# seanome/kmerseek

Hardware: AMD Instinct MI355X
Metric: k-mers hashed+matched/sec (higher is better)
Workload: dtype u64

## Files before the change

### include/kmerseek_amd.h

```cpp
#ifndef KMERSEEK_AMD_H
#define KMERSEEK_AMD_H

#include <stddef.h>
#include <stdint.h>

#ifdef __cplusplus
extern "C" {
#endif

#define KS_ABI_VERSION 1

typedef enum ks_status {
    KS_OK = 0,
    KS_ERR_INVALID_MOLTYPE = 1,
    KS_ERR_INVALID_KSIZE = 2,
    KS_ERR_INVALID_RESIDUE = 3,
    KS_ERR_INVALID_ARG = 4,
    KS_ERR_OOM = 5,
    KS_ERR_HIP = 6,
    KS_ERR_NO_DEVICE = 7,
    KS_ERR_CAPACITY = 8,
    KS_ERR_INVALID_SCALED = 9
} ks_status;

// ... 26 lines not shown
const char *ks_status_string(int status);

int ks_moltype_from_string(const char *name, uint32_t *moltype_out);

uint64_t ks_max_hash(uint32_t scaled);

int ks_ctx_create(int device, void *hip_stream, ks_ctx **out);
void ks_ctx_destroy(ks_ctx *ctx);
const char *ks_last_error(const ks_ctx *ctx);
void *ks_ctx_stream(const ks_ctx *ctx);
int ks_ctx_synchronize(ks_ctx *ctx);
int ks_ctx_pool_stats(const ks_ctx *ctx, uint64_t *n_blocks, uint64_t *bytes_held, uint64_t *bytes_in_use,
                      uint64_t *n_mallocs);

int ks_ctx_sketch_stats(const ks_ctx *ctx, uint64_t out[4]);
int ks_ctx_search_stats(const ks_ctx *ctx, uint64_t out[4]);
int ks_ctx_fused_stats(const ks_ctx *ctx, uint64_t out[3]);
int ks_ctx_qfilter_stats(const ks_ctx *ctx, uint64_t out[2]);
int ks_ctx_reload_debug_env(ks_ctx *ctx);
int ks_debug_guard_selftest(const char *what);

int ks_dev_malloc(ks_ctx *ctx, uint64_t bytes, void **out);
int ks_dev_free(ks_ctx *ctx, void *ptr);
int ks_dev_upload(ks_ctx *ctx, void *dst_device, const void *src_host, uint64_t bytes);
int ks_dev_download(ks_ctx *ctx, void *dst_host, const void *src_device, uint64_t bytes);

int ks_host_alloc(ks_ctx *ctx, uint64_t bytes, void **out);
int ks_host_free(ks_ctx *ctx, void *ptr);


typedef struct ks_residue_error {
    uint32_t seq_index;
// ... 535 lines not shown
```

### kmerseek_amd/_lib.py

```python
from __future__ import annotations

import ctypes as C
import os
import sys

HERE = os.path.dirname(os.path.abspath(__file__))
SO_PATH = os.environ.get("KMERSEEK_AMD_LIB") or os.path.join(HERE, "libkmerseek_amd.so")

KS_OK = 0
KS_ERR_INVALID_MOLTYPE = 1
KS_ERR_INVALID_KSIZE = 2
KS_ERR_INVALID_RESIDUE = 3
KS_ERR_INVALID_ARG = 4
KS_ERR_OOM = 5
KS_ERR_HIP = 6
KS_ERR_NO_DEVICE = 7
KS_ERR_CAPACITY = 8
KS_ERR_INVALID_SCALED = 9

KS_PROTEIN, KS_DAYHOFF, KS_HP = 0, 1, 2
KS_SEED_DEFAULT = 42


class ks_params(C.Structure):
# ... 119 lines not shown
_u64p = C.POINTER(C.c_uint64)
_pp = C.POINTER(C.c_void_p)
_parp = C.POINTER(ks_params)

SIGNATURES = {
    "ks_abi_version": (C.c_uint32, []),
    "ks_status_string": (C.c_char_p, [C.c_int]),
    "ks_moltype_from_string": (C.c_int, [C.c_char_p, _u32p]),
    "ks_max_hash": (C.c_uint64, [C.c_uint32]),
    "ks_ctx_create": (C.c_int, [C.c_int, _vp, _pp]),
    "ks_ctx_destroy": (None, [_vp]),
    "ks_last_error": (C.c_char_p, [_vp]),
    "ks_ctx_stream": (_vp, [_vp]),
    "ks_ctx_synchronize": (C.c_int, [_vp]),
    "ks_ctx_sketch_stats": (C.c_int, [_vp, C.POINTER(C.c_uint64 * 4)]),
    "ks_ctx_search_stats": (C.c_int, [_vp, C.POINTER(C.c_uint64 * 4)]),
    "ks_ctx_fused_stats": (C.c_int, [_vp, C.POINTER(C.c_uint64 * 3)]),
    "ks_ctx_qfilter_stats": (C.c_int, [_vp, C.POINTER(C.c_uint64 * 2)]),
    "ks_ctx_reload_debug_env": (C.c_int, [_vp]),
    "ks_debug_guard_selftest": (C.c_int, [C.c_char_p]),
    "ks_host_alloc": (C.c_int, [_vp, C.c_uint64, _pp]),
    "ks_host_free": (C.c_int, [_vp, _vp]),
    "ks_dev_malloc": (C.c_int, [_vp, C.c_uint64, _pp]),
    "ks_dev_free": (C.c_int, [_vp, _vp]),
    "ks_dev_upload": (C.c_int, [_vp, _vp, _vp, C.c_uint64]),
    "ks_dev_download": (C.c_int, [_vp, _vp, _vp, C.c_uint64]),
    "ks_ctx_pool_stats": (C.c_int, [_vp, _u64p, _u64p, _u64p, _u64p]),
    "ks_validate_and_resolve": (C.c_int, [C.c_char_p, C.c_uint64, C.c_int, C.c_uint64, C.c_char_p, _u64p,
                                          C.POINTER(ks_residue_error)]),
    "ks_sketch_batch": (C.c_int, [_vp, _vp, _vp, C.c_uint32, _parp, _pp]),
    "ks_sketch_batch_device": (C.c_int, [_vp, _vp, _vp, C.c_uint32, C.c_uint64, C.c_uint32, _parp, _pp]),
    "ks_sketch_queries_device": (C.c_int, [_vp, _vp, _vp, _vp, C.c_uint32, C.c_uint64, C.c_uint32, _pp]),
# ... 302 lines not shown
```

### kmerseek_amd/csrc/ks_api.hip

```cpp
#include "ks_device.h"

extern "C" int ks_sketch_batch_device(ks_ctx *ctx, const uint8_t *d_residues, const uint64_t *d_seq_offsets,
                                      uint32_t n_seqs, uint64_t n_residues, uint32_t max_seq_len,
                                      const ks_params *params, ks_sketches **out) {
    return ks_guard(ctx, [&]() -> int {
    if (!ctx) return KS_ERR_INVALID_ARG;
    if (!out || (!d_seq_offsets) || (!d_residues && n_residues)) return ks_fail(ctx, KS_ERR_INVALID_ARG, "NULL argument");
    return ks_sketch_device_impl(ctx, d_residues, d_seq_offsets, n_seqs, n_residues, max_seq_len, params, 0, 0, 0, out);
    });
}

extern "C" int ks_sketch_queries_device(ks_ctx *ctx, const ks_index *index, const uint8_t *d_residues,
                                        const uint64_t *d_seq_offsets, uint32_t n_seqs, uint64_t n_residues,
                                        uint32_t max_seq_len, ks_sketches **out) {
    return ks_guard(ctx, [&]() -> int {
    if (!ctx) return KS_ERR_INVALID_ARG;
    if (!index || !out || (!d_seq_offsets) || (!d_residues && n_residues)) return ks_fail(ctx, KS_ERR_INVALID_ARG, "NULL argument");
    return ks_sketch_device_impl(ctx, d_residues, d_seq_offsets, n_seqs, n_residues, max_seq_len, &index->params,
                                 index->pbits, (index->fp_layout && index->fp_shift == 32 - index->pbits) ? 1 : 0, 0, out);
    });
}

struct ks_upload {
    ks_ctx *ctx;
// ... 246 lines not shown
    if (!ctx) return KS_ERR_INVALID_ARG;
    return ks_index_build_impl(ctx, targets, out);
    });
}
extern "C" uint32_t ks_index_n_targets(const ks_index *ix) { return ix ? ix->n_targets : 0; }
extern "C" uint64_t ks_index_n_postings(const ks_index *ix) { return ix ? ix->n_postings : 0; }
extern "C" void ks_index_free(ks_index *ix) {
    if (!ix) return;
    ks_pool_free(ix->ctx, ix->d_keys);
    ks_pool_free(ix->ctx, ix->d_tids);
    ks_pool_free(ix->ctx, ix->d_abunds);
    ks_pool_free(ix->ctx, ix->d_fp);
    ks_pool_free(ix->ctx, ix->d_post);
    ks_pool_free(ix->ctx, ix->d_bmeta);
    ks_pool_free(ix->ctx, ix->d_presence);
    ks_pool_free(ix->ctx, ix->d_dir);
    delete ix;
}

extern "C" int ks_search(ks_ctx *ctx, const ks_index *index, const ks_sketches *queries, ks_hits **out) {
    return ks_guard(ctx, [&]() -> int {
    if (!ctx) return KS_ERR_INVALID_ARG;
    return ks_search_impl(ctx, index, queries, out);
    });
}
extern "C" int ks_search_ex(ks_ctx *ctx, const ks_index *index, const ks_sketches *queries, const ks_search_opts *opts, ks_hits **out) {
    return ks_guard(ctx, [&]() -> int {
    KS_TRY(ks_search_opts_check(ctx, opts));
    if (!ctx) return KS_ERR_INVALID_ARG;
    return ks_search_impl(ctx, index, queries, out, nullptr, opts);
    });
}
static int sketch_search_impl(ks_ctx *ctx, const ks_index *index, const uint8_t *d_residues, const uint64_t *d_seq_offsets, uint32_t n_seqs,
                              uint64_t n_residues, uint32_t max_seq_len, const ks_search_opts *opts, ks_sketches **sketches_out,
                              ks_hits **hits_out) {
    *hits_out = nullptr;
    if (sketches_out) *sketches_out = nullptr;
    const int fmt10 = (index->fp_layout && index->fp_shift == 32 - index->pbits) ? 1 : 0;
    ks_sketches *S = nullptr;
    ks_hits *H = nullptr;
    const u64 agg_before = ctx->agg_used;
    int st = ks_sketch_device_impl(ctx, d_residues, d_seq_offsets, n_seqs, n_residues, max_seq_len, &index->params, index->pbits, fmt10,
                                   ks_dbg(ctx, KS_DBG_NO_DEFER) ? 0 : 1, &S);
    if (st != KS_OK) return st;
    const bool deferred = S->pending != 0;
    int redo = 0;
    st = ks_search_impl(ctx, index, S, &H, &redo, opts);
    if (S->pending) {
        const ks_fetch_seg f = ks_sketch_pending_seg(S);
        int r2 = 0;
        int st2 = ks_stream_wait_fetch(ctx, &f, 1);
        if (st2 == KS_OK) st2 = ks_sketch_finish_pending(S, &r2);
        if (st == KS_OK) { st = st2; redo = r2; }
    }
    if (st == KS_OK && redo) {
        ks_hits_free(H); H = nullptr;
        ks_sketches_free(S); S = nullptr;
        ctx->fused_redos++;
        st = ks_sketch_device_impl(ctx, d_residues, d_seq_offsets, n_seqs, n_residues, max_seq_len, &index->params, index->pbits, fmt10, 0, &S);
        if (st == KS_OK) st = ks_search_impl(ctx, index, S, &H, nullptr, opts);
    }
    if (st != KS_OK) { ks_hits_free(H); ks_sketches_free(S); return st; }
    if (deferred) ctx->fused_deferred++;
    if (ctx->agg_used > agg_before) ctx->fused_aggregated++;
    *hits_out = H;
    if (sketches_out) *sketches_out = S; else ks_sketches_free(S);
    return KS_OK;
}

extern "C" int ks_sketch_search_device_ex(ks_ctx *ctx, const ks_index *index, const uint8_t *d_residues,
                                          const uint64_t *d_seq_offsets, uint32_t n_seqs, uint64_t n_residues,
                                          uint32_t max_seq_len, const ks_search_opts *opts, ks_sketches **sketches_out,
                                          ks_hits **hits_out) {
    return ks_guard(ctx, [&]() -> int {
    KS_TRY(ks_search_opts_check(ctx, opts));
    if (!ctx) return KS_ERR_INVALID_ARG;
    if (!index || !hits_out || (!d_seq_offsets) || (!d_residues && n_residues)) return ks_fail(ctx, KS_ERR_INVALID_ARG, "NULL argument");
    return sketch_search_impl(ctx, index, d_residues, d_seq_offsets, n_seqs, n_residues, max_seq_len, opts, sketches_out, hits_out);
    });
// ... 670 lines not shown
```

### kmerseek_amd/csrc/ks_common.h

```cpp
#pragma once

#include <hip/hip_runtime.h>

#include <cstdint>
#include <cstdio>
#include <cstring>
#include <functional>
#include <initializer_list>
#include <new>
#include <stdexcept>
#include <string>
#include <vector>

#include "../../include/kmerseek_amd.h"

typedef uint8_t u8;
typedef uint16_t u16;
typedef uint32_t u32;
typedef uint64_t u64;
typedef int32_t i32;
typedef int64_t i64;

#define KS_WAVE 64

// ... 46 lines not shown
    std::vector<std::pair<hipEvent_t, hipEvent_t>> t_free;
    bool t_open = false;
    u64 *h_pin = nullptr;
    u64 pair_cap_hint = 0;
    u64 rows_hint = 0;
    bool sketch_use_ticket = false;
    u64 sketch_ticket_fallbacks = 0, sketch_compact_fallbacks = 0, sketch_cap_fallbacks = 0;
    bool rows_use_ticket = false; u64 rows_ticket_fallbacks = 0;
    u64 fused_deferred = 0, fused_redos = 0;
    u64 fused_aggregated = 0;
    u64 join_retries = 0;
    double rows_mult = 0.0;
    u64 agg_used = 0, agg_overflows = 0, agg_oflow_rows = 0;
    bool qfilter_pays = true;
    u64 qfilter_seen = 0, qfilter_dropped = 0;
    unsigned long long *scan_ring = nullptr;
    u32 *scan_ticket = nullptr;
    u32 scan_ticket_base = 0;
    u8 *d_lut = nullptr;
    unsigned long long *h_flag = nullptr;
    unsigned long long wait_seq = 0;
};

int ks_stream_wait(ks_ctx *ctx);
#define KS_FETCH_MAX 4
struct ks_fetch_seg {
    const void *src;
    u32 *dst;
    u32 rows, row_words, src_stride;
};
// ... 203 lines not shown
    u64 n_postings;
    u64 *d_keys;
    u32 *d_tids;
    u32 *d_abunds;
    u32 *d_fp;
    ks_post *d_post;
    ks_bmeta *d_bmeta;
    bool fp_layout;
    int fp_shift;
    u32 max_abund;
    u64 *d_dir;
    int pbits;
    u32 *d_presence;
    u32 pres_K;
    int pres_bits;
};

struct rf_cols {
    const u32 *qid, *tid, *isect;
    const u64 *nw, *median2;
    const double *ss;
};

enum : u32 { KS_COLS_RANKED = 1u, KS_COLS_GATHER = 2u };
struct ks_hit_cols {
    u32 *d_qid, *d_tid, *d_isect;
    u64 *d_nw;
    u64 *d_block;
    u64 *d_median2;
    double *d_ss;
// ... 294 lines not shown
```

### kmerseek_amd/csrc/ks_ctx.hip

```cpp
#include <cstdarg>
#include <algorithm>

#include "ks_common.h"

int ks_fail(ks_ctx *ctx, int status, const char *fmt, ...) {
    char buf[512];
    va_list ap;
    va_start(ap, fmt);
    vsnprintf(buf, sizeof buf, fmt, ap);
    va_end(ap);
    if (ctx) {
        try { ctx->err = buf; } catch (...) { }
    }
    return status;
}

extern "C" uint32_t ks_abi_version(void) { return KS_ABI_VERSION; }


bool ks_same_params(const ks_params &a, const ks_params &b) {
    return a.ksize == b.ksize && a.scaled == b.scaled && a.moltype == b.moltype && a.seed == b.seed && a.flags == b.flags;
}
int ks_params_check_same(ks_ctx *ctx, const char *pass, const char *noun, const ks_params &a, const ks_params &b) {
    if (ks_same_params(a, b)) return KS_OK;
// ... 165 lines not shown
    if (bytes_in_use) *bytes_in_use = used;
    if (n_mallocs) *n_mallocs = ctx->pool_mallocs;
    return KS_OK;
    });
}

extern "C" int ks_ctx_sketch_stats(const ks_ctx *ctx, uint64_t out[4]) {
    return ks_guard((ks_ctx *)ctx, [&]() -> int {
    if (!ctx || !out) return KS_ERR_INVALID_ARG;
    out[0] = ctx->sketch_ticket_fallbacks; out[1] = ctx->sketch_use_ticket ? 1 : 0;
    out[2] = ctx->sketch_compact_fallbacks; out[3] = ctx->sketch_cap_fallbacks;
    return KS_OK;
    });
}

extern "C" int ks_ctx_search_stats(const ks_ctx *ctx, uint64_t out[4]) {
    return ks_guard((ks_ctx *)ctx, [&]() -> int {
    if (!ctx || !out) return KS_ERR_INVALID_ARG;
    out[0] = ctx->join_retries; out[1] = ctx->rows_ticket_fallbacks;
    out[2] = ctx->agg_used; out[3] = ctx->agg_overflows;
    return KS_OK;
    });
}

extern "C" int ks_ctx_qfilter_stats(const ks_ctx *ctx, uint64_t out[2]) {
    return ks_guard((ks_ctx *)ctx, [&]() -> int {
    if (!ctx || !out) return KS_ERR_INVALID_ARG;
    out[0] = ctx->qfilter_seen; out[1] = ctx->qfilter_dropped;
    return KS_OK;
    });
}

extern "C" int ks_ctx_fused_stats(const ks_ctx *ctx, uint64_t out[3]) {
    return ks_guard((ks_ctx *)ctx, [&]() -> int {
    if (!ctx || !out) return KS_ERR_INVALID_ARG;
    out[0] = ctx->fused_deferred; out[1] = ctx->fused_redos; out[2] = ctx->fused_aggregated;
    return KS_OK;
    });
}

extern "C" int ks_dev_malloc(ks_ctx *ctx, uint64_t bytes, void **out) {
    return ks_guard(ctx, [&]() -> int {
    if (!ctx || !out) return KS_ERR_INVALID_ARG;
    KS_HIP(ctx, hipSetDevice(ctx->device));
    if (hipMalloc(out, bytes ? bytes : 256) != hipSuccess) { (void)hipGetLastError(); return ks_fail(ctx, KS_ERR_OOM, "hipMalloc(%llu) failed", (unsigned long long)bytes); }
    return KS_OK;
    });
}
extern "C" int ks_dev_free(ks_ctx *ctx, void *ptr) {
    return ks_guard(ctx, [&]() -> int {
    if (!ctx) return KS_ERR_INVALID_ARG;
// ... 350 lines not shown
```

### kmerseek_amd/csrc/ks_device.h

```cpp
#pragma once
#include "ks_common.h"

#define KS_DEV __device__ __forceinline__

KS_DEV u64 ks_rotl64(u64 x, int r) {
#ifndef KS_NO_OPAQUE
    if (__builtin_constant_p(r) && r > 0 && r < 64 && r != 32) {
        const u32 lo = (u32)x, hi = (u32)(x >> 32);
        const u32 s = (u32)(r < 32 ? 32 - r : 64 - r);
        const u32 a = __builtin_amdgcn_alignbit(lo, hi, s), b = __builtin_amdgcn_alignbit(hi, lo, s);
        return r < 32 ? (((u64)b << 32) | a) : (((u64)a << 32) | b);
    }
#endif
    return (x << r) | (x >> (64 - r));
}

KS_DEV u64 ks_fmix64(u64 k) {
    k ^= k >> 33;
    k *= 0xff51afd7ed558ccdULL;
    k ^= k >> 33;
    k *= 0xc4ceb9fe1a85ec53ULL;
    k ^= k >> 33;
    return k;
}
// ... 337 lines not shown
    u32 plo = ~0u, phi = ~0u;
#pragma unroll
    for (int b = 0; b < 8; b++) {
        const u32 bm = (u32)__builtin_amdgcn_sbfe((int)d, (u32)b, 1u);
        const u64 m = __ballot(bm != 0u);
        plo &= ~((u32)m ^ bm);
        phi &= ~((u32)(m >> 32) ^ bm);
    }
    const u32 below = __builtin_amdgcn_mbcnt_hi(phi, __builtin_amdgcn_mbcnt_lo(plo, 0));
    const u32 pre = wc[d];
    if (below == 0) wc[d] = pre + (u32)__popc(plo) + (u32)__popc(phi);
    return (d << 16) | (pre + below);
}

KS_DEV u32 ks_join_prefix(u64 h, u32 K) { return __umulhi((u32)(h >> 32), K); }
KS_DEV u32 ks_rs_digit(u64 key, int shift, u32 K) {
    return K ? ((ks_join_prefix(key, K) >> shift) & 255u) : ((u32)(key >> shift) & 255u);
}
```

### kmerseek_amd/csrc/ks_prims.hip

```cpp
#include "ks_device.h"
#include <type_traits>

template <typename T>
KS_DEV T wave_incl_scan_t(T v) {
    const u32 lane = threadIdx.x & 63;
#pragma unroll
    for (int d = 1; d < 64; d <<= 1) {
        T t = __shfl_up(v, d, 64);
        if (lane >= (u32)d) v += t;
    }
    return v;
}

template <typename T>
KS_DEV T block_excl_scan_t(T v, T *smem , T *total) {
    const u32 lane = threadIdx.x & 63, wave = threadIdx.x >> 6, nw = blockDim.x >> 6;
    T incl = wave_incl_scan_t<T>(v);
    if (lane == 63) smem[wave] = incl;
    __syncthreads();
    if (wave == 0) {
        T w = lane < nw ? smem[lane] : (T)0;
        T wi = wave_incl_scan_t<T>(w);
        if (lane < nw) smem[lane] = wi - w;
        if (lane == nw - 1) smem[nw] = wi;
// ... 365 lines not shown
        const u64 len = seg_len[r], off = (u64)j * RS_TILE;
        nvalid = off < len ? (u32)((len - off) < RS_TILE ? (len - off) : RS_TILE) : 0u;
        tile_base = (u64)r * seg_cap + off;
    }
    if (nvalid == 0) return;
    const u32 region = (bid / tiles_per_seg) >> sub_shift;
    if (tid < BKS_NB) cnt[tid] = 0;
    u64 key[RS_IPT];
    u32 val[RS_IPT];
    u32 rank[RS_IPT];
#pragma unroll
    for (int r = 0; r < RS_IPT; r++) {
        const u32 li = (u32)r * RS_THREADS + tid;
        const bool valid = li < nvalid;
        key[r] = valid ? kin[tile_base + li] : 0ULL;
        val[r] = valid ? (V16 ? (u32)((const u16 *)vin)[tile_base + li] : vin[tile_base + li]) : 0u;
    }
    __syncthreads();
    const bool full = !QF && nvalid == RS_TILE;
    if constexpr (QF) {
        u32 bit[RS_IPT], dg[RS_IPT];
#pragma unroll
        for (int r = 0; r < RS_IPT; r++) {
            u32 hh = (u32)(key[r] >> 32);
            if (V16) hh = (hh & ~(0xffu << fix_s)) | (region << fix_s);
            bit[r] = __umulhi(hh, presK);
        }
        u32 w[RS_IPT];
#pragma unroll
        for (int r = 0; r < RS_IPT; r++) w[r] = presence[bit[r] >> 5];
#pragma unroll
        for (int r = 0; r < RS_IPT; r++) {
            const bool live = (u32)r * RS_THREADS + tid < nvalid && ((w[r] >> (bit[r] & 31u)) & 1u);
            dg[r] = live ? ((ks_join_prefix(key[r], pfxK) >> shift) & (n_hi - 1u)) : (u32)BKS_NB + (tid & 63u);
        }
#pragma unroll
        for (int r = 0; r < RS_IPT; r++) rank[r] = atomicAdd(&cnt[dg[r]], 1u);
#pragma unroll
        for (int r = 0; r < RS_IPT; r++) rank[r] = dg[r] < BKS_NB ? (rank[r] | (dg[r] << 16)) : 0xffffffffu;
    } else if (full) {
        u32 dg[RS_IPT];
#pragma unroll
        for (int r = 0; r < RS_IPT; r++) dg[r] = (ks_join_prefix(key[r], pfxK) >> shift) & (n_hi - 1u);
#pragma unroll
        for (int r = 0; r < RS_IPT; r++) rank[r] = atomicAdd(&cnt[dg[r]], 1u);
#pragma unroll
        for (int r = 0; r < RS_IPT; r++) rank[r] |= dg[r] << 16;
    } else {
#pragma unroll
// ... 69 lines not shown
                const u64 k = ks_[i];
                const u64 g = (u64)KS_BSLOT(dd[i], region, n_hi) * bcap + sl[i];
                if (V16 == 2) {
                    const u32 v = vo[V16 == 2 ? i : 0];
                    kout[g] = (k & ~(0xffULL << 56)) | ((u64)(v & 0xffu) << 56);
                    ((u8 *)vout)[g] = (u8)(v >> 8);
                } else {
                    kout[g] = k;
                }
            }
        }
    }
    if (V16 == 2) return;
    __syncthreads();
    u32 *vstage = (u32 *)stage;
    if (full) {
#pragma unroll
        for (int r = 0; r < RS_IPT; r++) vstage[rank[r]] = val[r];
    } else {
#pragma unroll
        for (int r = 0; r < RS_IPT; r++)
            if (rank[r] != 0xffffffffu) vstage[rank[r]] = val[r];
    }
    __syncthreads();
#pragma unroll
    for (int i = 0; i < RS_IPT; i++)
        if (sl[i] != 0xffffffffu) {
            const u64 g = (u64)KS_BSLOT(dd[i], region, n_hi) * bcap + sl[i];
            if (V16) ((u16 *)vout)[g] = (u16)vstage[(u32)i * RS_THREADS + tid];
            else vout[g] = vstage[(u32)i * RS_THREADS + tid];
// ... 323 lines not shown
```

### kmerseek_amd/csrc/ks_search.hip

```cpp
#include "ks_device.h"

__global__ __launch_bounds__(256) void k_fill_index_vals(const u64 *csr, const u32 *abunds, u32 n_seqs, u64 *vals) {
    const u32 s = blockIdx.x * 4 + (threadIdx.x >> 6);
    if (s >= n_seqs) return;
    const u64 b = csr[s], e = csr[s + 1];
    for (u64 j = b + (threadIdx.x & 63); j < e; j += 64) vals[j] = ((u64)abunds[j] << 32) | s;
}

__global__ __launch_bounds__(256) void k_fill_query_vals(const u64 *csr, u32 n_seqs, u32 *vals) {
    const u32 s = blockIdx.x * 4 + (threadIdx.x >> 6);
    if (s >= n_seqs) return;
    const u64 b = csr[s], e = csr[s + 1];
    for (u64 j = b + (threadIdx.x & 63); j < e; j += 64) vals[j] = s;
}

__global__ __launch_bounds__(256) void k_split_vals(const u64 *vals, u64 n, u32 *tids, u32 *abunds, u32 *max_abund) {
    u64 i = (u64)blockIdx.x * blockDim.x + threadIdx.x;
    u32 a = 0;
    if (i < n) {
        u64 v = vals[i];
        tids[i] = (u32)v;
        a = (u32)(v >> 32);
        abunds[i] = a;
    }
// ... 1 lines not shown
        const u32 o = __shfl_down(a, d, 64);
        a = o > a ? o : a;
    }
    if ((threadIdx.x & 63) == 0 && a > *max_abund) atomicMax(max_abund, a);
}

int ks_join_pbits(const ks_ctx *ctx, u64 n_postings, u64 per_bucket);
__global__ __launch_bounds__(256) void k_bucket_dir(const u64 *keys, u64 n, int pbits, u32 pfxK, u64 *dir);
__global__ __launch_bounds__(256) void k_index_finish(const u64 *keys, const u32 *tids, const u32 *abunds, const u64 *dir, u64 n, int pbits,
                                                      u32 pfxK, int fp_shift, u32 *fp, ks_post *post);
__global__ __launch_bounds__(256) void k_index_bmeta(const u64 *keys, const u64 *dir, u32 n_buckets, int fp_shift, ks_bmeta *bmeta);

__global__ __launch_bounds__(256) void k_index_presence(const u64 *keys, u64 n, u32 presK, u32 *presence) {
    const u64 i = (u64)blockIdx.x * 256 + threadIdx.x;
    if (i >= n) return;
    const u32 b = ks_join_prefix(keys[i], presK);
    if (i > 0 && ks_join_prefix(keys[i - 1], presK) == b) return;
    atomicOr(&presence[b >> 5], 1u << (b & 31u));
}
#define KS_QF_OCC 3
static int presence_bits(const ks_ctx *ctx, u64 n_postings, int pbits) {
    u64 occ = KS_QF_OCC;
    if (const char *f = ks_dbg(ctx, KS_DBG_QFILTER_OCC)) { const long v = atol(f); if (v >= 1 && v <= 64) occ = (u64)v; }
    int bits = pbits;
    while (bits < 31 && (1ULL << bits) < occ * n_postings) bits++;
    return bits;
}

#define JN_FP_PBITS 15

static int index_build_run(ks_ctx *ctx, const ks_sketches *t, ks_index *ix) {
    const u64 n = t->n_hashes;
    u64 *k0 = nullptr, *k1 = nullptr, *v0 = nullptr, *v1 = nullptr;
    u32 *d_max = nullptr;
    ks_scratch sc(ctx);
    KS_TRY(sc.alloc(&v0, (size_t)n));
    KS_TRY(ks_alloc(ctx, &ix->d_tids, (size_t)n));
    KS_TRY(ks_alloc(ctx, &ix->d_abunds, (size_t)n));
    KS_TRY(sc.alloc(&d_max, 1));
    KS_HIP(ctx, hipMemsetAsync(d_max, 0, sizeof(u32), ctx->stream));
    if (n > 0) {
// ... 41 lines not shown
        if (ix->fp_layout) {
            KS_TRY(ks_alloc(ctx, &ix->d_fp, (size_t)(n ? n : 1)));
            KS_TRY(ks_alloc(ctx, &ix->d_post, (size_t)(n ? n : 1)));
            ix->fp_shift = 32 - ix->pbits;
            if (ks_dbg(ctx, KS_DBG_FP_COARSEN)) {
                ix->fp_shift += atoi(ks_dbg(ctx, KS_DBG_FP_COARSEN));
                if (ix->fp_shift > 63) ix->fp_shift = 63;
            }
            KS_TRY(ks_alloc(ctx, &ix->d_bmeta, (size_t)nb));
            hipLaunchKernelGGL(k_index_bmeta, dim3((nb + 255) / 256), dim3(256), 0, ctx->stream, (const u64 *)ix->d_keys, (const u64 *)ix->d_dir,
                               nb, ix->fp_shift, ix->d_bmeta);
            KS_HIP(ctx, hipGetLastError());
            if (n > 0)
                KS_LAUNCH(ctx, "index_finish", k_index_finish, (u32)((n + 255) / 256), 256, (const u64 *)ix->d_keys, (const u32 *)ix->d_tids,
                          (const u32 *)ix->d_abunds, (const u64 *)ix->d_dir, n, ix->pbits, K, ix->fp_shift, ix->d_fp, ix->d_post);
            ix->pres_bits = presence_bits(ctx, n, ix->pbits);
            ix->pres_K = ks_join_prefix_mul(ix->pres_bits, ks_max_hash(t->params.scaled));
            const size_t pres_words = ix->pres_bits > 5 ? (size_t)1 << (ix->pres_bits - 5) : 1;
            KS_TRY(ks_alloc(ctx, &ix->d_presence, pres_words));
            KS_HIP(ctx, hipMemsetAsync(ix->d_presence, 0, pres_words * sizeof(u32), ctx->stream));
            if (n > 0)
                KS_LAUNCH(ctx, "index_presence", k_index_presence, (u32)((n + 255) / 256), 256, (const u64 *)ix->d_keys, n, ix->pres_K,
                          ix->d_presence);
        }
    }
    KS_TRY(ks_scan_status_fetch(ctx));
    KS_HIP(ctx, hipStreamSynchronize(ctx->stream));
    KS_TRY(ks_scan_status_check(ctx));
    if (ix->fp_layout) {
        ks_pool_free(ctx, ix->d_keys); ks_pool_free(ctx, ix->d_tids); ks_pool_free(ctx, ix->d_abunds);
        ix->d_keys = nullptr; ix->d_tids = nullptr; ix->d_abunds = nullptr;
    }
    return KS_OK;
}

int ks_index_build_impl(ks_ctx *ctx, const ks_sketches *t, ks_index **out) {
    if (!t || !out) return ks_fail(ctx, KS_ERR_INVALID_ARG, "NULL argument");
    KS_HIP(ctx, hipSetDevice(ctx->device));
// ... 773 lines not shown
        const u64 i = i0 + (u64)j * 256 + threadIdx.x;
        if (i < n) dk[i] = kk[j];
    }
}


struct se_search {
    const ks_index *ix;
    const ks_sketches *q;
    u64 n_q;
    int pbits, tbits, qbits, abits;
    u32 n_buckets, pfxK;
    bool pre, f10;
    bool qf;
    u64 qf_kept;
    u64 *dir_q;
    unsigned long long *cursor;
    u32 *bcur;
    u64 *pk0, *pk1;
    u64 n_pairs, seg_cap, seg_count[JN_SEGS];
    u32 n_segs;
    bool stop;
    bool stats;
    double min_c;
};
static_assert(2 * JN_SEGS <= KS_PIN_JOIN_WORDS, "pinned slot of the join's segment counts");

struct se_qview {
    u64 *qk;
    u32 *qv;
// ... 27 lines not shown
    const int pbits = Q.pbits;
    const u32 n_buckets = Q.n_buckets;
    memset(V, 0, sizeof *V);
    if (way == 1 && Q.f10) Q.pre = false;
    const u32 q_s = (way == 0 && Q.f10) ? q->part_s : 0u;
    V->q_fmt = q_s ? ((pbits == 16 && q_s == 48u && !ks_dbg(ctx, KS_DBG_POSTINGS10)) ? 2 : 1) : 0;
    KS_HIP(ctx, hipMemsetAsync(Q.cursor, 0, ((size_t)JN_SEGS * JN_CUR_STRIDE + (way == 0 ? (n_buckets + 1) / 2 : 0)) * sizeof(u64), ctx->stream));
    if (way == 0) {
        const u64 per = Q.n_q / n_buckets;
        const u32 bcap = (u32)(per + per / 8 + 512);
        KS_TRY(sc.alloc(&V->qk0, (size_t)n_buckets * bcap));
        KS_TRY(sc.alloc(&V->qv0, (size_t)n_buckets * bcap));
        ks_rs_segments seg{q->part_len, q->part_cap, q->part_regions << q->part_sub_shift, q->part_sub_shift};
        const char *qf_knob = ks_dbg(ctx, KS_DBG_QFILTER);
        Q.qf = Q.ix->d_presence && (qf_knob ? atoi(qf_knob) != 0 : ctx->qfilter_pays);
        KS_TRY(ks_bucket_scatter_u32(ctx, q->part_keys, q->part_vals, &seg, 8, Q.pfxK, V->qk0, V->qv0, Q.bcur, bcap, Q.cursor, n_buckets >> 8,
                                     V->q_fmt,
                                     Q.qf ? Q.ix->d_presence : nullptr, Q.ix->pres_K, q_s ? q_s - 32u : 0u));
        V->bucket_posting_bytes = V->q_fmt == 2 ? 9 : (V->q_fmt == 1 ? 10 : 12);
        KS_LAUNCH(ctx, "bucket_dir", k_region_dir, (n_buckets + 255) / 256, 256, (const u32 *)Q.bcur, (u64)bcap, n_buckets, Q.dir_q,
                  Q.dir_q + n_buckets, n_buckets >> 8);
        V->qk = V->qk0; V->qv = V->qv0; V->q_lo = Q.dir_q; V->q_hi = Q.dir_q + n_buckets;
        V->partition_path = 1;
    } else if (Q.pre && pbits <= 8) {
        V->qk = q->part_keys; V->qv = q->part_vals;
        KS_LAUNCH(ctx, "bucket_dir", k_region_dir, (n_buckets + 255) / 256, 256, (const u32 *)q->part_len, q->part_cap, n_buckets, Q.dir_q,
                  Q.dir_q + n_buckets, 0u);
        V->q_lo = Q.dir_q; V->q_hi = Q.dir_q + n_buckets;
        V->partition_path = 0;
    } else {
        const u64 n_q = Q.n_q;
        if (!Q.pre) KS_TRY(ks_sketches_make_dense(ctx, const_cast<ks_sketches *>(q)));
        KS_TRY(sc.alloc(&V->qk0, (size_t)n_q)); KS_TRY(sc.alloc(&V->qk1, (size_t)n_q));
// ... 23 lines not shown
    const ks_index *ix = Q.ix;
    const u32 n_buckets = Q.n_buckets;
    const int q_fmt = V.q_fmt;
    *overflowed = false;
    {
        const u64 per_bucket = Q.n_q / n_buckets, round = (u64)JN_THREADS * JN_E;
        const u64 reservations = (u64)n_buckets * ((per_bucket + round - 1) / round ? (per_bucket + round - 1) / round : 1);
        Q.n_segs = (ix->fp_layout && reservations >= 8192 && n_buckets >= JN_SEGS && !ks_dbg(ctx, KS_DBG_ONE_CURSOR)) ? JN_SEGS : 1;
        if (ix->fp_layout && ks_dbg(ctx, KS_DBG_JOIN_SEGS) && n_buckets >= JN_SEGS) Q.n_segs = JN_SEGS;
    }
    const u32 n_segs = Q.n_segs;
    Q.seg_cap = n_segs == 1 ? cap : cap / n_segs + cap / n_segs / 8 + 4096;
    if (ks_dbg(ctx, KS_DBG_JOIN_SEG_CAP)) Q.seg_cap = strtoull(ks_dbg(ctx, KS_DBG_JOIN_SEG_CAP), nullptr, 10);
    const u64 *dir_t = ix->d_dir;
    const u64 *pin = ctx->h_pin + KS_PIN_JOIN;
    for (int attempt = 0; attempt < 2; attempt++) {
        const u64 seg_cap = Q.seg_cap;
        KS_TRY(sc.alloc(&Q.pk0, (size_t)(seg_cap * n_segs)));
        if (attempt > 0)
            KS_HIP(ctx, hipMemset2DAsync(Q.cursor, (size_t)JN_CUR_STRIDE * sizeof(u64), 0, sizeof(u64), JN_SEGS, ctx->stream));
        const bool sparse = ix->fp_layout && (ks_dbg(ctx, KS_DBG_JOIN_SPARSE) ? atoi(ks_dbg(ctx, KS_DBG_JOIN_SPARSE)) != 0
                                                                             : Q.n_q / n_buckets <= (u64)JS_QCAP * 3 / 4);
        if (sparse)
            KS_LAUNCH(ctx, "join_buckets", (q_fmt == 2 ? k_join_sparse<2> : (q_fmt ? k_join_sparse<1> : k_join_sparse<0>)), n_buckets, JS_THREADS,
                      (const u64 *)V.qk, (const u32 *)V.qv, (const u32 *)ix->d_fp, (const ks_post *)ix->d_post, (const ks_bmeta *)ix->d_bmeta,
                      V.q_lo, V.q_hi, dir_t, Q.pk0, seg_cap, Q.cursor, n_segs - 1, Q.tbits, Q.abits, ix->fp_shift);
        else if (ix->fp_layout)
            KS_LAUNCH(ctx, "join_buckets", (q_fmt == 2 ? k_join_buckets<2> : (q_fmt ? k_join_buckets<1> : k_join_buckets<0>)), n_buckets, JN_THREADS,
                      (const u64 *)V.qk, (const u32 *)V.qv, (const u32 *)ix->d_fp, (const ks_post *)ix->d_post, (const ks_bmeta *)ix->d_bmeta,
                      V.q_lo, V.q_hi, dir_t, Q.pk0, seg_cap, Q.cursor, n_segs - 1, Q.tbits, Q.abits, ix->fp_shift);
        else {
            u32 split = 1;
            if (ctx->pair_cap_hint > Q.n_q && Q.n_q / n_buckets >= 1024) {
                const u64 dens2 = 2 * ctx->pair_cap_hint / Q.n_q;
                split = dens2 >= 6 ? 4u : (dens2 >= 3 ? 2u : 1u);
            }
            if (const char *f = ks_dbg(ctx, KS_DBG_JOIN_SPLIT)) { const int v = atoi(f); if (v >= 1 && v <= 16) split = (u32)v; }
// ... 136 lines not shown
        KS_TRY(se_wait_pending(ctx, Q, sketch_redo));
        if ((*stop = Q.stop)) return KS_OK;
    }
    u64 cap = Q.n_q < (1u << 20) ? (1u << 20) : Q.n_q;
    if (ctx->pair_cap_hint > cap) cap = ctx->pair_cap_hint;
    for (int way = (Q.pre && Q.pbits > 8) ? 0 : 1; way < 2; way++) {
        se_qview V;
        KS_TRY(se_partition(ctx, Q, way, sc, &V));
        if (V.bucket_posting_bytes) H->bucket_posting_bytes = V.bucket_posting_bytes;
        bool overflowed = false;
        KS_TRY(se_join(ctx, Q, V, way, cap, sc, &split->pairs, sketch_redo, &overflowed));
        if ((*stop = Q.stop)) return KS_OK;
        sc.free(V.qk0); sc.free(V.qk1); sc.free(V.qv0); sc.free(V.qv1);
        if (!overflowed) {
            H->partition_path = V.partition_path;
            if (way == 0 && Q.qf) {
                const u64 dropped = Q.n_q > Q.qf_kept ? Q.n_q - Q.qf_kept : 0;
                ctx->qfilter_seen += Q.n_q;
                ctx->qfilter_dropped += dropped;
                ctx->qfilter_pays = dropped >= Q.n_q / 2;
            } else if (way == 0 && ix->d_presence && Q.n_pairs < Q.n_q / 4) {
                ctx->qfilter_pays = true;
            }
            break;
        }
        sc.free(Q.pk0); Q.pk0 = nullptr;
    }
    H->n_pair_instances = Q.n_pairs;
    const u64 want = Q.n_pairs + Q.n_pairs / 8;
    ctx->pair_cap_hint = want > ctx->pair_cap_hint / 2 ? want : ctx->pair_cap_hint / 2;
    u64 *pk = nullptr;
    struct agg_plan : ks_msd_plan {
        ks_ctx *c;
        explicit agg_plan(ks_ctx *c_) : ks_msd_plan{}, c(c_) {}
// ... 103 lines not shown
```

### kmerseek_amd/engine.py

```python
from __future__ import annotations

import ctypes as C
from typing import Dict, List, Optional, Sequence, Tuple

import numpy as np

from . import _lib
from ._lib import ks_params

MOLTYPES = {"protein": _lib.KS_PROTEIN, "raw": _lib.KS_PROTEIN, "dayhoff": _lib.KS_DAYHOFF, "hp": _lib.KS_HP}
MOLTYPE_NAMES = {_lib.KS_PROTEIN: "protein", _lib.KS_DAYHOFF: "dayhoff", _lib.KS_HP: "hp"}
SEED = _lib.KS_SEED_DEFAULT


class KmerseekError(RuntimeError):
    def __init__(self, status: int, message: str):
        super().__init__(message)
        self.status = status


class InvalidAminoAcid(KmerseekError):

    def __init__(self, char: str, position: int, seq_index: int = 0):
        super().__init__(_lib.KS_ERR_INVALID_RESIDUE, f"Invalid amino acid '{char}' found at position {position}")
# ... 182 lines not shown
    def unpack_hits64_device(self, d_packed: int, n: int, qbits: int, tbits: int, d_qid: int, d_tid: int, d_isect: int, d_nw: int):
        self._check(self._L.ks_hits_unpack64_device(self._h, C.c_void_p(d_packed), n, qbits, tbits, C.c_void_p(d_qid), C.c_void_p(d_tid),
                                                    C.c_void_p(d_isect), C.c_void_p(d_nw)))

    def merge_hits_by_qid_device(self, d_qid: int, d_tid: int, d_isect: int, d_nw: int, block_rows: Sequence[int], n_queries: int,
                                 o_qid: int, o_tid: int, o_isect: int, o_nw: int):
        rows = (C.c_uint64 * len(block_rows))(*[int(x) for x in block_rows])
        self._check(self._L.ks_hits_merge_by_qid_device(self._h, C.c_void_p(d_qid), C.c_void_p(d_tid), C.c_void_p(d_isect), C.c_void_p(d_nw),
                                                        rows, len(block_rows), int(n_queries), C.c_void_p(o_qid), C.c_void_p(o_tid),
                                                        C.c_void_p(o_isect), C.c_void_p(o_nw)))

    def reload_debug_env(self):
        self._check(self._L.ks_ctx_reload_debug_env(self._h))

    def search_stats(self, paths: bool = False) -> Dict[str, int]:
        v = (C.c_uint64 * 4)()
        self._check(self._L.ks_ctx_search_stats(self._h, C.byref(v)))
        out = {"join_retries": int(v[0]), "rows_ticket_fallbacks": int(v[1]), "agg_overflows": int(v[3])}
        if paths:
            out["agg_used"] = int(v[2])
        return out

    def sketch_batch(self, residues: np.ndarray, offsets: np.ndarray, ksize: int, scaled: int, moltype: str,
                     seed: int = SEED) -> "Sketches":
        residues = np.ascontiguousarray(residues, dtype=np.uint8)
        offsets = np.ascontiguousarray(offsets, dtype=np.uint64)
        p = make_params(ksize, scaled, moltype, seed)
        out = C.c_void_p()
        self._check(self._L.ks_sketch_batch(self._h, _ptr(residues), _ptr(offsets), len(offsets) - 1, C.byref(p),
                                            C.byref(out)))
        return Sketches(self, out)

    def sketch_batch_device(self, d_residues: int, d_offsets: int, n_seqs: int, n_residues: int, ksize: int,
                            scaled: int, moltype: str, max_seq_len: int = 0, seed: int = SEED) -> "Sketches":
        p = make_params(ksize, scaled, moltype, seed)
# ... 67 lines not shown

    def sketch_translated_device(self, d_nt: int, d_offsets: int, n_seqs: int, n_nt: int, ksize: int, scaled: int, moltype: str,
                                 max_seq_len: int = 0, seed: int = SEED) -> "Sketches":
        p = make_params(ksize, scaled, moltype, seed)
        out = C.c_void_p()
        self._check(self._L.ks_sketch_translated_device(self._h, C.c_void_p(d_nt), C.c_void_p(d_offsets), n_seqs, n_nt, max_seq_len,
                                                        C.byref(p), C.byref(out)))
        return Sketches(self, out)

    def qfilter_stats(self) -> Dict[str, int]:
        v = (C.c_uint64 * 2)()
        self._check(self._L.ks_ctx_qfilter_stats(self._h, C.byref(v)))
        return {"seen": int(v[0]), "dropped": int(v[1])}

    def fused_stats(self) -> Dict[str, int]:
        v = (C.c_uint64 * 3)()
        self._check(self._L.ks_ctx_fused_stats(self._h, C.byref(v)))
        return {"deferred": int(v[0]), "redos": int(v[1]), "aggregated": int(v[2])}

    def sketches_from_host(self, offsets: np.ndarray, hashes: np.ndarray, abunds: np.ndarray, ksize: int,
                           scaled: int, moltype: str, seed: int = SEED) -> "Sketches":
        offsets = np.ascontiguousarray(offsets, dtype=np.uint64)
        hashes = np.ascontiguousarray(hashes, dtype=np.uint64)
        abunds = np.ascontiguousarray(abunds, dtype=np.uint32)
        p = make_params(ksize, scaled, moltype, seed)
        out = C.c_void_p()
        self._check(self._L.ks_sketches_from_host(self._h, _ptr(offsets), _ptr(hashes), _ptr(abunds),
                                                  len(offsets) - 1, C.byref(p), C.byref(out)))
        return Sketches(self, out)

    def kmer_positions(self, residues: np.ndarray, offsets: np.ndarray, ksize: int, scaled: int, moltype: str,
                       seed: int = SEED) -> Tuple[np.ndarray, np.ndarray, np.ndarray]:
        residues = np.ascontiguousarray(residues, dtype=np.uint8)
# ... 1148 lines not shown
```

Baseline: 61.25 billion.

## Sharpen query presence filter with second bit, larger table, and filter-aware join choice

The presence filter now sets and tests two bits per key (prefix bit plus a hash-derived bit within the word), which lowers false positives so fewer non-matching query k-mers get scattered and joined. A second, larger presence table is built at index time and used when buckets would be dense. Sparse-versus-dense join selection now uses the keep ratio of the previous query filter instead of the raw query count. Value loads in the filtered scatter are deferred until after filtering, so dropped keys skip them. The cost is extra index memory, an extra build pass, and reliance on the previous call's filter ratio, which can misjudge the join choice when batches differ.

```diff
diff --git a/include/kmerseek_amd.h b/include/kmerseek_amd.h
--- a/include/kmerseek_amd.h
+++ b/include/kmerseek_amd.h
@@ -64,8 +64,8 @@
                       uint64_t *n_mallocs);
 
 int ks_ctx_sketch_stats(const ks_ctx *ctx, uint64_t out[4]);
-int ks_ctx_search_stats(const ks_ctx *ctx, uint64_t out[4]);
-int ks_ctx_fused_stats(const ks_ctx *ctx, uint64_t out[3]);
+int ks_ctx_search_stats(const ks_ctx *ctx, uint64_t out[5]);
+int ks_ctx_fused_stats(const ks_ctx *ctx, uint64_t out[4]);
 int ks_ctx_qfilter_stats(const ks_ctx *ctx, uint64_t out[2]);
 int ks_ctx_reload_debug_env(ks_ctx *ctx);
 int ks_debug_guard_selftest(const char *what);
diff --git a/kmerseek_amd/_lib.py b/kmerseek_amd/_lib.py
--- a/kmerseek_amd/_lib.py
+++ b/kmerseek_amd/_lib.py
@@ -157,8 +157,8 @@
     "ks_ctx_stream": (_vp, [_vp]),
     "ks_ctx_synchronize": (C.c_int, [_vp]),
     "ks_ctx_sketch_stats": (C.c_int, [_vp, C.POINTER(C.c_uint64 * 4)]),
-    "ks_ctx_search_stats": (C.c_int, [_vp, C.POINTER(C.c_uint64 * 4)]),
-    "ks_ctx_fused_stats": (C.c_int, [_vp, C.POINTER(C.c_uint64 * 3)]),
+    "ks_ctx_search_stats": (C.c_int, [_vp, C.POINTER(C.c_uint64 * 5)]),
+    "ks_ctx_fused_stats": (C.c_int, [_vp, C.POINTER(C.c_uint64 * 4)]),
     "ks_ctx_qfilter_stats": (C.c_int, [_vp, C.POINTER(C.c_uint64 * 2)]),
     "ks_ctx_reload_debug_env": (C.c_int, [_vp]),
     "ks_debug_guard_selftest": (C.c_int, [C.c_char_p]),
diff --git a/kmerseek_amd/csrc/ks_api.hip b/kmerseek_amd/csrc/ks_api.hip
--- a/kmerseek_amd/csrc/ks_api.hip
+++ b/kmerseek_amd/csrc/ks_api.hip
@@ -284,6 +284,7 @@
     ks_pool_free(ix->ctx, ix->d_post);
     ks_pool_free(ix->ctx, ix->d_bmeta);
     ks_pool_free(ix->ctx, ix->d_presence);
+    ks_pool_free(ix->ctx, ix->d_presence_big);
     ks_pool_free(ix->ctx, ix->d_dir);
     delete ix;
 }
@@ -309,7 +310,7 @@
     const int fmt10 = (index->fp_layout && index->fp_shift == 32 - index->pbits) ? 1 : 0;
     ks_sketches *S = nullptr;
     ks_hits *H = nullptr;
-    const u64 agg_before = ctx->agg_used;
+    const u64 agg_before = ctx->agg_used, table_before = ctx->join_table;
     int st = ks_sketch_device_impl(ctx, d_residues, d_seq_offsets, n_seqs, n_residues, max_seq_len, &index->params, index->pbits, fmt10,
                                    ks_dbg(ctx, KS_DBG_NO_DEFER) ? 0 : 1, &S);
     if (st != KS_OK) return st;
@@ -333,6 +334,7 @@
     if (st != KS_OK) { ks_hits_free(H); ks_sketches_free(S); return st; }
     if (deferred) ctx->fused_deferred++;
     if (ctx->agg_used > agg_before) ctx->fused_aggregated++;
+    if (ctx->join_table > table_before) ctx->fused_table_joined++;
     *hits_out = H;
     if (sketches_out) *sketches_out = S; else ks_sketches_free(S);
     return KS_OK;
diff --git a/kmerseek_amd/csrc/ks_common.h b/kmerseek_amd/csrc/ks_common.h
--- a/kmerseek_amd/csrc/ks_common.h
+++ b/kmerseek_amd/csrc/ks_common.h
@@ -84,6 +84,8 @@
     u64 agg_used = 0, agg_overflows = 0, agg_oflow_rows = 0;
     bool qfilter_pays = true;
     u64 qfilter_seen = 0, qfilter_dropped = 0;
+    u64 qf_last_seen = 0, qf_last_kept = 0;
+    u64 join_table = 0, fused_table_joined = 0;
     unsigned long long *scan_ring = nullptr;
     u32 *scan_ticket = nullptr;
     u32 scan_ticket_base = 0;
@@ -317,6 +319,9 @@
     u32 *d_presence;
     u32 pres_K;
     int pres_bits;
+    u32 *d_presence_big;
+    u32 pres_big_K;
+    int pres_big_bits;
 };
 
 struct rf_cols {
diff --git a/kmerseek_amd/csrc/ks_ctx.hip b/kmerseek_amd/csrc/ks_ctx.hip
--- a/kmerseek_amd/csrc/ks_ctx.hip
+++ b/kmerseek_amd/csrc/ks_ctx.hip
@@ -203,11 +203,12 @@
     });
 }
 
-extern "C" int ks_ctx_search_stats(const ks_ctx *ctx, uint64_t out[4]) {
+extern "C" int ks_ctx_search_stats(const ks_ctx *ctx, uint64_t out[5]) {
     return ks_guard((ks_ctx *)ctx, [&]() -> int {
     if (!ctx || !out) return KS_ERR_INVALID_ARG;
     out[0] = ctx->join_retries; out[1] = ctx->rows_ticket_fallbacks;
     out[2] = ctx->agg_used; out[3] = ctx->agg_overflows;
+    out[4] = ctx->join_table;
     return KS_OK;
     });
 }
@@ -220,10 +221,11 @@
     });
 }
 
-extern "C" int ks_ctx_fused_stats(const ks_ctx *ctx, uint64_t out[3]) {
+extern "C" int ks_ctx_fused_stats(const ks_ctx *ctx, uint64_t out[4]) {
     return ks_guard((ks_ctx *)ctx, [&]() -> int {
     if (!ctx || !out) return KS_ERR_INVALID_ARG;
     out[0] = ctx->fused_deferred; out[1] = ctx->fused_redos; out[2] = ctx->fused_aggregated;
+    out[3] = ctx->fused_table_joined;
     return KS_OK;
     });
 }
diff --git a/kmerseek_amd/csrc/ks_device.h b/kmerseek_amd/csrc/ks_device.h
--- a/kmerseek_amd/csrc/ks_device.h
+++ b/kmerseek_amd/csrc/ks_device.h
@@ -375,6 +375,7 @@
 }
 
 KS_DEV u32 ks_join_prefix(u64 h, u32 K) { return __umulhi((u32)(h >> 32), K); }
+KS_DEV u32 ks_presence_bit2(u64 h) { return ((u32)h >> 8) & 31u; }
 KS_DEV u32 ks_rs_digit(u64 key, int shift, u32 K) {
     return K ? ((ks_join_prefix(key, K) >> shift) & 255u) : ((u32)(key >> shift) & 255u);
 }
diff --git a/kmerseek_amd/csrc/ks_prims.hip b/kmerseek_amd/csrc/ks_prims.hip
--- a/kmerseek_amd/csrc/ks_prims.hip
+++ b/kmerseek_amd/csrc/ks_prims.hip
@@ -403,7 +403,7 @@
         const u32 li = (u32)r * RS_THREADS + tid;
         const bool valid = li < nvalid;
         key[r] = valid ? kin[tile_base + li] : 0ULL;
-        val[r] = valid ? (V16 ? (u32)((const u16 *)vin)[tile_base + li] : vin[tile_base + li]) : 0u;
+        if (!QF || V16 == 2) val[r] = valid ? (V16 ? (u32)((const u16 *)vin)[tile_base + li] : vin[tile_base + li]) : 0u;
     }
     __syncthreads();
     const bool full = !QF && nvalid == RS_TILE;
@@ -419,9 +419,19 @@
 #pragma unroll
         for (int r = 0; r < RS_IPT; r++) w[r] = presence[bit[r] >> 5];
 #pragma unroll
+        for (int r = 0; r < RS_IPT; r++)
+            bit[r] = (1u << (bit[r] & 31u)) | (1u << ks_presence_bit2(key[r]));
+#pragma unroll
         for (int r = 0; r < RS_IPT; r++) {
-            const bool live = (u32)r * RS_THREADS + tid < nvalid && ((w[r] >> (bit[r] & 31u)) & 1u);
+            const bool live = (u32)r * RS_THREADS + tid < nvalid && (w[r] & bit[r]) == bit[r];
             dg[r] = live ? ((ks_join_prefix(key[r], pfxK) >> shift) & (n_hi - 1u)) : (u32)BKS_NB + (tid & 63u);
+        }
+        if (V16 == 1) {
+#pragma unroll
+            for (int r = 0; r < RS_IPT; r++) {
+                const u32 li = (u32)r * RS_THREADS + tid;
+                val[r] = li < nvalid ? (u32)((const u16 *)vin)[tile_base + li] : 0u;
+            }
         }
 #pragma unroll
         for (int r = 0; r < RS_IPT; r++) rank[r] = atomicAdd(&cnt[dg[r]], 1u);
@@ -521,6 +531,10 @@
     if (V16 == 2) return;
     __syncthreads();
     u32 *vstage = (u32 *)stage;
+    if constexpr (QF && V16 == 0) {
+#pragma unroll
+        for (int r = 0; r < RS_IPT; r++) val[r] = rank[r] != 0xffffffffu ? vin[tile_base + (u32)r * RS_THREADS + tid] : 0u;
+    }
     if (full) {
 #pragma unroll
         for (int r = 0; r < RS_IPT; r++) vstage[rank[r]] = val[r];
diff --git a/kmerseek_amd/csrc/ks_search.hip b/kmerseek_amd/csrc/ks_search.hip
--- a/kmerseek_amd/csrc/ks_search.hip
+++ b/kmerseek_amd/csrc/ks_search.hip
@@ -39,17 +39,25 @@
 __global__ __launch_bounds__(256) void k_index_presence(const u64 *keys, u64 n, u32 presK, u32 *presence) {
     const u64 i = (u64)blockIdx.x * 256 + threadIdx.x;
     if (i >= n) return;
-    const u32 b = ks_join_prefix(keys[i], presK);
-    if (i > 0 && ks_join_prefix(keys[i - 1], presK) == b) return;
-    atomicOr(&presence[b >> 5], 1u << (b & 31u));
+    const u64 k = keys[i];
+    if (i > 0 && keys[i - 1] == k) return;
+    const u32 b = ks_join_prefix(k, presK);
+    atomicOr(&presence[b >> 5], (1u << (b & 31u)) | (1u << ks_presence_bit2(k)));
 }
 #define KS_QF_OCC 3
-static int presence_bits(const ks_ctx *ctx, u64 n_postings, int pbits) {
-    u64 occ = KS_QF_OCC;
-    if (const char *f = ks_dbg(ctx, KS_DBG_QFILTER_OCC)) { const long v = atol(f); if (v >= 1 && v <= 64) occ = (u64)v; }
+#define KS_QF_OCC_BIG 6
+static int presence_bits(u64 occ, u64 n_postings, int pbits) {
     int bits = pbits;
     while (bits < 31 && (1ULL << bits) < occ * n_postings) bits++;
     return bits;
+}
+static int presence_build(ks_ctx *ctx, const u64 *d_keys, u64 n, int bits, u64 max_hash, u32 **out, u32 *out_K) {
+    *out_K = ks_join_prefix_mul(bits, max_hash);
+    const size_t words = bits > 5 ? (size_t)1 << (bits - 5) : 1;
+    KS_TRY(ks_alloc(ctx, out, words));
+    KS_HIP(ctx, hipMemsetAsync(*out, 0, words * sizeof(u32), ctx->stream));
+    if (n > 0) KS_LAUNCH(ctx, "index_presence", k_index_presence, (u32)((n + 255) / 256), 256, d_keys, n, *out_K, *out);
+    return KS_OK;
 }
 
 #define JN_FP_PBITS 15
@@ -121,14 +129,14 @@
             if (n > 0)
                 KS_LAUNCH(ctx, "index_finish", k_index_finish, (u32)((n + 255) / 256), 256, (const u64 *)ix->d_keys, (const u32 *)ix->d_tids,
                           (const u32 *)ix->d_abunds, (const u64 *)ix->d_dir, n, ix->pbits, K, ix->fp_shift, ix->d_fp, ix->d_post);
-            ix->pres_bits = presence_bits(ctx, n, ix->pbits);
-            ix->pres_K = ks_join_prefix_mul(ix->pres_bits, ks_max_hash(t->params.scaled));
-            const size_t pres_words = ix->pres_bits > 5 ? (size_t)1 << (ix->pres_bits - 5) : 1;
-            KS_TRY(ks_alloc(ctx, &ix->d_presence, pres_words));
-            KS_HIP(ctx, hipMemsetAsync(ix->d_presence, 0, pres_words * sizeof(u32), ctx->stream));
-            if (n > 0)
-                KS_LAUNCH(ctx, "index_presence", k_index_presence, (u32)((n + 255) / 256), 256, (const u64 *)ix->d_keys, n, ix->pres_K,
-                          ix->d_presence);
+            u64 occ = KS_QF_OCC, occ_big = KS_QF_OCC_BIG;
+            if (const char *f = ks_dbg(ctx, KS_DBG_QFILTER_OCC)) { const long v = atol(f); if (v >= 1 && v <= 64) occ = occ_big = (u64)v; }
+            const u64 mh = ks_max_hash(t->params.scaled);
+            ix->pres_bits = presence_bits(occ, n, ix->pbits);
+            KS_TRY(presence_build(ctx, (const u64 *)ix->d_keys, n, ix->pres_bits, mh, &ix->d_presence, &ix->pres_K));
+            ix->pres_big_bits = presence_bits(occ_big, n, ix->pbits);
+            if (ix->pres_big_bits > ix->pres_bits)
+                KS_TRY(presence_build(ctx, (const u64 *)ix->d_keys, n, ix->pres_big_bits, mh, &ix->d_presence_big, &ix->pres_big_K));
         }
     }
     KS_TRY(ks_scan_status_fetch(ctx));
@@ -932,6 +940,7 @@
     bool pre, f10;
     bool qf;
     u64 qf_kept;
+    bool table;
     u64 *dir_q;
     unsigned long long *cursor;
     u32 *bcur;
@@ -989,9 +998,11 @@
         ks_rs_segments seg{q->part_len, q->part_cap, q->part_regions << q->part_sub_shift, q->part_sub_shift};
         const char *qf_knob = ks_dbg(ctx, KS_DBG_QFILTER);
         Q.qf = Q.ix->d_presence && (qf_knob ? atoi(qf_knob) != 0 : ctx->qfilter_pays);
+        const bool big = Q.ix->d_presence_big && Q.n_q / n_buckets > (u64)JS_QCAP * 3 / 4;
         KS_TRY(ks_bucket_scatter_u32(ctx, q->part_keys, q->part_vals, &seg, 8, Q.pfxK, V->qk0, V->qv0, Q.bcur, bcap, Q.cursor, n_buckets >> 8,
                                      V->q_fmt,
-                                     Q.qf ? Q.ix->d_presence : nullptr, Q.ix->pres_K, q_s ? q_s - 32u : 0u));
+                                     Q.qf ? (big ? Q.ix->d_presence_big : Q.ix->d_presence) : nullptr, big ? Q.ix->pres_big_K : Q.ix->pres_K,
+                                     q_s ? q_s - 32u : 0u));
         V->bucket_posting_bytes = V->q_fmt == 2 ? 9 : (V->q_fmt == 1 ? 10 : 12);
         KS_LAUNCH(ctx, "bucket_dir", k_region_dir, (n_buckets + 255) / 256, 256, (const u32 *)Q.bcur, (u64)bcap, n_buckets, Q.dir_q,
                   Q.dir_q + n_buckets, n_buckets >> 8);
@@ -1045,13 +1056,17 @@
     if (ks_dbg(ctx, KS_DBG_JOIN_SEG_CAP)) Q.seg_cap = strtoull(ks_dbg(ctx, KS_DBG_JOIN_SEG_CAP), nullptr, 10);
     const u64 *dir_t = ix->d_dir;
     const u64 *pin = ctx->h_pin + KS_PIN_JOIN;
+    u64 fill = Q.n_q / n_buckets;
+    if (way == 0 && Q.qf && ctx->qf_last_seen)
+        fill = (u64)((double)Q.n_q * ((double)ctx->qf_last_kept / (double)ctx->qf_last_seen)) / n_buckets;
+    const bool sparse = ix->fp_layout && (ks_dbg(ctx, KS_DBG_JOIN_SPARSE) ? atoi(ks_dbg(ctx, KS_DBG_JOIN_SPARSE)) != 0
+                                                                         : fill <= (u64)JS_QCAP * 3 / 4);
+    Q.table = sparse;
     for (int attempt = 0; attempt < 2; attempt++) {
         const u64 seg_cap = Q.seg_cap;
         KS_TRY(sc.alloc(&Q.pk0, (size_t)(seg_cap * n_segs)));
         if (attempt > 0)
             KS_HIP(ctx, hipMemset2DAsync(Q.cursor, (size_t)JN_CUR_STRIDE * sizeof(u64), 0, sizeof(u64), JN_SEGS, ctx->stream));
-        const bool sparse = ix->fp_layout && (ks_dbg(ctx, KS_DBG_JOIN_SPARSE) ? atoi(ks_dbg(ctx, KS_DBG_JOIN_SPARSE)) != 0
-                                                                             : Q.n_q / n_buckets <= (u64)JS_QCAP * 3 / 4);
         if (sparse)
             KS_LAUNCH(ctx, "join_buckets", (q_fmt == 2 ? k_join_sparse<2> : (q_fmt ? k_join_sparse<1> : k_join_sparse<0>)), n_buckets, JS_THREADS,
                       (const u64 *)V.qk, (const u32 *)V.qv, (const u32 *)ix->d_fp, (const ks_post *)ix->d_post, (const ks_bmeta *)ix->d_bmeta,
@@ -1218,10 +1233,13 @@
         sc.free(V.qk0); sc.free(V.qk1); sc.free(V.qv0); sc.free(V.qv1);
         if (!overflowed) {
             H->partition_path = V.partition_path;
+            if (Q.table) ctx->join_table++;
             if (way == 0 && Q.qf) {
                 const u64 dropped = Q.n_q > Q.qf_kept ? Q.n_q - Q.qf_kept : 0;
                 ctx->qfilter_seen += Q.n_q;
                 ctx->qfilter_dropped += dropped;
+                ctx->qf_last_seen = Q.n_q;
+                ctx->qf_last_kept = Q.n_q - dropped;
                 ctx->qfilter_pays = dropped >= Q.n_q / 2;
             } else if (way == 0 && ix->d_presence && Q.n_pairs < Q.n_q / 4) {
                 ctx->qfilter_pays = true;
diff --git a/kmerseek_amd/engine.py b/kmerseek_amd/engine.py
--- a/kmerseek_amd/engine.py
+++ b/kmerseek_amd/engine.py
@@ -220,11 +220,12 @@
         self._check(self._L.ks_ctx_reload_debug_env(self._h))
 
     def search_stats(self, paths: bool = False) -> Dict[str, int]:
-        v = (C.c_uint64 * 4)()
+        v = (C.c_uint64 * 5)()
         self._check(self._L.ks_ctx_search_stats(self._h, C.byref(v)))
         out = {"join_retries": int(v[0]), "rows_ticket_fallbacks": int(v[1]), "agg_overflows": int(v[3])}
         if paths:
             out["agg_used"] = int(v[2])
+            out["join_table"] = int(v[4])
         return out
 
     def sketch_batch(self, residues: np.ndarray, offsets: np.ndarray, ksize: int, scaled: int, moltype: str,
@@ -322,9 +323,9 @@
         return {"seen": int(v[0]), "dropped": int(v[1])}
 
     def fused_stats(self) -> Dict[str, int]:
-        v = (C.c_uint64 * 3)()
+        v = (C.c_uint64 * 4)()
         self._check(self._L.ks_ctx_fused_stats(self._h, C.byref(v)))
-        return {"deferred": int(v[0]), "redos": int(v[1]), "aggregated": int(v[2])}
+        return {"deferred": int(v[0]), "redos": int(v[1]), "aggregated": int(v[2]), "table_joined": int(v[3])}
 
     def sketches_from_host(self, offsets: np.ndarray, hashes: np.ndarray, abunds: np.ndarray, ksize: int,
                            scaled: int, moltype: str, seed: int = SEED) -> "Sketches":
```

Result: faster. 63.12 billion (median of 6 runs) (+3.1%).
